# capnproto/capnproto-rust

Measured on AMD Instinct MI355X. Metric: GiB/s packed encode+decode, device-resident segments; % HBM roofline, higher is better.
Workload: dtype u8; 1 GPU; config2: 1048576 segments x 1024 B per GPU, ~30 % zero words, pack+unpack round trip; segments_per_gpu=1048576, unpacked_bytes_per_gpu=1073741824, global_unpacked_bytes=1073741824, parallelism=shard1

## Files before the change

capnproto-rust_amd/csrc/capi.hip:

```cpp
#ifndef CAPNP_STATE_ALLOC
#define CAPNP_STATE_ALLOC 1
#endif
#include <hip/hip_runtime.h>

#include <stdint.h>
#include <stdio.h>
#include <string.h>

#include <algorithm>
#include <chrono>
#include <string>
#include <cmath>
#include <mutex>
#include <vector>

#include "../../include/capnp_packed.h"
#include "../../include/capnp_packed_bench.h"
#include "common.h"
#include "frame.h"

extern "C" hipError_t capnp_launch_pack(const uint64_t*, const uint64_t*, uint64_t, uint32_t,
                                        uint8_t*, uint64_t, uint64_t*, uint64_t*, uint32_t*,
                                        hipStream_t);
extern "C" hipError_t capnp_launch_pack_gap(const uint64_t*, const uint64_t*, uint64_t, uint32_t,
                                            uint8_t*, uint64_t, uint64_t*, uint64_t*,
                                            const uint32_t*, hipStream_t);
extern "C" uint32_t capnp_pack_tile_words(void);
extern "C" hipError_t capnp_launch_msg_gap(const uint64_t*, const uint64_t*, uint64_t, uint64_t,
                                           uint32_t*, uint32_t*, hipStream_t);
extern "C" hipError_t capnp_launch_msg_tables(const uint64_t*, const uint64_t*, uint64_t,
                                              const uint64_t*, uint8_t*, uint64_t, uint64_t*,
                                              hipStream_t);
extern "C" hipError_t capnp_msg_scan_bytes(uint64_t, size_t*);
extern "C" hipError_t capnp_launch_msg_prepare(const uint64_t*, const uint64_t*, const uint64_t*,
                                               uint64_t, uint64_t*, uint64_t*, uint64_t*,
                                               uint64_t*, void*, size_t, uint64_t*, uint64_t*,
                                               hipStream_t);
extern "C" hipError_t capnp_launch_msg_offsets(const uint64_t*, const uint64_t*, uint64_t,
                                               uint64_t*, hipStream_t);
extern "C" hipError_t capnp_launch_msg_frame(const uint8_t*, const uint64_t*, uint64_t, int,
                                             uint64_t, int, uint64_t*, uint64_t*, int32_t*,
                                             uint64_t*, void*, size_t, uint64_t*, uint64_t*,
                                             hipStream_t);
extern "C" hipError_t capnp_launch_msg_segs(const uint8_t*, const uint64_t*, uint64_t, int,
                                            uint64_t, int, const int32_t*, const uint64_t*,
                                            const uint64_t*, const uint64_t*, uint64_t*,
                                            uint64_t*, uint64_t*, hipStream_t);
extern "C" hipError_t capnp_launch_msg_status(uint64_t, const int32_t*, const uint64_t*,
                                              const int32_t*, const uint64_t*, int32_t*,
                                              uint64_t*, hipStream_t);
extern "C" hipError_t capnp_launch_flat_frame(const uint8_t*, const uint64_t*, uint64_t, int,
                                              uint64_t, int, uint64_t*, int32_t*, uint64_t*,
                                              uint64_t*, void*, size_t, uint64_t*, hipStream_t);
extern "C" hipError_t capnp_launch_flat_segs(const uint8_t*, const uint64_t*, uint64_t, int,
                                             uint64_t, int, const int32_t*, const uint64_t*,
                                             uint32_t*, hipStream_t);
extern "C" size_t capnp_pack_state_bytes(uint64_t, uint32_t);
extern "C" hipError_t capnp_launch_unpack(const uint8_t*, const uint64_t*, uint64_t, uint32_t,
                                          uint64_t*, const uint64_t*, int32_t*, uint64_t*,
                                          const uint32_t*, hipStream_t);
extern "C" hipError_t capnp_launch_gen(uint64_t*, const uint64_t*, uint64_t, uint64_t,
                                       const uint8_t*, uint32_t, uint32_t, hipStream_t);
extern "C" uint64_t capnp_carsales_plan(const uint32_t*, uint64_t, uint64_t, uint32_t*, uint64_t*,
                                        uint64_t);
extern "C" hipError_t capnp_launch_gen_carsales(uint64_t*, uint64_t, const uint32_t*,
                                                const uint64_t*, uint64_t, hipStream_t);
extern "C" size_t capnp_resync_ws_bytes(uint64_t n, uint64_t total_bytes);
extern "C" size_t capnp_msg_chain_ws_bytes(uint64_t words_cap);
extern "C" hipError_t capnp_resync_read_stream(const uint8_t*, uint64_t, uint64_t, uint64_t*,
                                               uint64_t*, uint64_t, uint64_t*, uint64_t*,
                                               uint64_t*, int*, void*, size_t, hipStream_t,
                                               uint64_t*);
extern "C" hipError_t capnp_launch_msg_meta(const uint64_t*, const uint64_t*, uint64_t, uint64_t,
                                            int, uint64_t*, uint64_t*, uint64_t*, hipStream_t);
extern "C" hipError_t capnp_launch_msg_seglist(const uint64_t*, const uint64_t*, uint64_t,
                                               const uint64_t*, uint64_t*, hipStream_t);
// ... 27 lines not shown
                                          uint64_t total_bytes, uint64_t* d_out,
                                          const uint64_t* d_out_off, int32_t* d_status,
                                          uint64_t* d_consumed, void* d_ws, size_t ws_bytes,
                                          hipStream_t s, int* passes, int* serial,
                                          const int32_t** failed_flag);
extern "C" hipError_t capnp_launch_msg_read(const uint8_t*, uint64_t, uint32_t, uint32_t, uint64_t,
                                            uint32_t, uint64_t, uint64_t, FrameResult*, uint64_t*,
                                            uint64_t*, uint32_t*, uint32_t, hipStream_t);
extern "C" uint32_t capnp_msg_pack_words(void);
extern "C" hipError_t capnp_launch_msg_pack(const uint64_t*, const uint64_t*, uint32_t, uint32_t,
                                            uint8_t*, uint64_t, uint64_t*, uint32_t*, uint32_t,
                                            uint8_t*, hipStream_t);
extern "C" hipError_t capnp_launch_frame(const uint8_t*, uint64_t, uint32_t, uint32_t, uint64_t,
                                         uint32_t, uint64_t, uint64_t, FrameResult*, hipStream_t);
extern "C" hipError_t capnp_launch_msg_read_service(const uint64_t*, uint64_t*, uint32_t, uint64_t,
                                                    FrameResult*, uint32_t*, hipStream_t);
extern "C" hipError_t capnp_launch_msg_pack_service(const uint64_t*, uint64_t*, uint32_t, uint64_t,
                                                    uint32_t*, hipStream_t);

namespace {

constexpr uint32_t kDefaultTileChunks = 16;
constexpr uint32_t kMaxTileChunks = 64;

size_t round16(size_t x) { return (x + 15) & ~size_t(15); }

}

constexpr size_t kTablePrefixBytes = 4096;
#ifndef PARALLEL_BODY_WORDS
#define PARALLEL_BODY_WORDS 65536
#endif
constexpr uint64_t kParallelBodyWords = PARALLEL_BODY_WORDS;

struct CallSvc {
    hipStream_t s = nullptr;
    uint64_t* h = nullptr;
    uint64_t* d = nullptr;
    uint64_t* line = nullptr;
    const uint64_t* line_d = nullptr;
    bool line_dev = false;
    uint64_t args[kSvcArgs] = {};
    uint64_t bell = 0;
    uint32_t gen = 0;
    bool live = false;
    std::chrono::steady_clock::time_point last{};
};

struct capnp_ctx {
    int device = 0;
    hipStream_t stream = nullptr;
    uint8_t* d_state = nullptr;
    size_t state_cap = 0;
    uint8_t* d_stage = nullptr;
    size_t stage_cap = 0;
    uint8_t* d_body = nullptr;
    size_t body_cap = 0;
    FrameResult* d_frame = nullptr;
    FrameResult* h_frame = nullptr;
    hipStream_t sstream[3] = {nullptr, nullptr, nullptr};
    hipEvent_t ev_in[2] = {}, ev_comp[2] = {}, ev_off[2] = {}, ev_out[2] = {};
    uint8_t* d_slot[2] = {nullptr, nullptr};
    size_t slot_cap = 0;
    uint64_t* h_slot_off[2] = {nullptr, nullptr};
    size_t h_slot_off_cap = 0;
    uint8_t* d_msg = nullptr;
    size_t msg_cap = 0;
    uint8_t* d_resync = nullptr;
    size_t resync_cap = 0;
    uint8_t* d_wt = nullptr;
    size_t wt_cap = 0;
    uint8_t* d_pwt = nullptr;
    size_t pwt_cap = 0;
    uint8_t* d_stream_words = nullptr;
    size_t stream_words_cap = 0;
    int resync_passes = 0, resync_serial = 0;
    const int32_t* resync_failed = nullptr;
    hipStream_t resync_stream = nullptr;
    hipEvent_t ev_resync = nullptr;
    uint32_t* d_bad = nullptr;
    uint32_t* h_bad = nullptr;
    uint8_t* h_pin = nullptr;
    uint8_t* d_pin = nullptr;
    size_t pin_cap = 0;
    FrameResult* d_hframe = nullptr;
    uint8_t* d_req = nullptr;
    int req_ok = -1;
    uint32_t* h_flag = nullptr;
    uint32_t* d_flag = nullptr;
    uint32_t call_seq = 0;
    CallSvc svc[2];
    std::chrono::steady_clock::time_point percall_last{};
    bool percall_any = false;
    static constexpr int kUseSlots = 8;
    hipStream_t use_s[kUseSlots] = {};
    hipEvent_t use_ev[kUseSlots] = {};
    int use_next = 0;
    std::string err;
};

constexpr size_t kPinnedCall = size_t(4) << 20;
#ifndef WRITE_PIN_MAX
#define WRITE_PIN_MAX kPinnedCall
#endif
constexpr size_t kWritePinMax = WRITE_PIN_MAX;

// ... 27 lines not shown
}

#define HIP_TRY(expr)                                   \
    do {                                                \
        hipError_t e_ = (expr);                         \
        if (e_ != hipSuccess) return fail(ctx, e_, #expr); \
    } while (0)

hipStream_t pick(capnp_ctx*, void* s) { return (hipStream_t)s; }

void mark_use(capnp_ctx* ctx, hipStream_t s) {
    if (s == ctx->stream) return;
    hipStreamCaptureStatus cs = hipStreamCaptureStatusNone;
    if (hipStreamIsCapturing(s, &cs) != hipSuccess || cs != hipStreamCaptureStatusNone) return;
    int k = 0;
    while (k < capnp_ctx::kUseSlots && !(ctx->use_ev[k] && ctx->use_s[k] == s)) k++;
    if (k == capnp_ctx::kUseSlots) {
        k = ctx->use_next;
        ctx->use_next = (k + 1) % capnp_ctx::kUseSlots;
        if (ctx->use_ev[k]) {
            (void)hipEventSynchronize(ctx->use_ev[k]);
        } else if (hipEventCreateWithFlags(&ctx->use_ev[k], hipEventDisableTiming) != hipSuccess) {
            ctx->use_ev[k] = nullptr;
            (void)hipStreamSynchronize(s);
            return;
        }
    }
    ctx->use_s[k] = s;
    if (hipEventRecord(ctx->use_ev[k], s) != hipSuccess) (void)hipStreamSynchronize(s);
}

struct UseMark {
    capnp_ctx* ctx;
    hipStream_t s;
    ~UseMark() {
        if (ctx) mark_use(ctx, s);
    }
};

void svc_stop_all(capnp_ctx* ctx);

hipError_t wait_uses(capnp_ctx* ctx) {
    svc_stop_all(ctx);
    hipError_t e = hipSuccess, r;
    if (ctx->stream && (r = hipStreamSynchronize(ctx->stream)) != hipSuccess) e = r;
    for (int k = 0; k < capnp_ctx::kUseSlots; k++)
        if (ctx->use_ev[k] && ctx->use_s[k] && (r = hipEventSynchronize(ctx->use_ev[k])) != hipSuccess)
            e = r;
    for (int k = 0; k < 3; k++)
        if (ctx->sstream[k] && (r = hipStreamSynchronize(ctx->sstream[k])) != hipSuccess) e = r;
    return e;
}

capnp_status ensure_state(capnp_ctx* ctx, size_t bytes) {
    if (bytes <= ctx->state_cap) return CAPNP_OK;
    HIP_TRY(hipSetDevice(ctx->device));
    if (ctx->d_state) {
        HIP_TRY(wait_uses(ctx));
        HIP_TRY(hipFree(ctx->d_state));
        ctx->d_state = nullptr;
        ctx->state_cap = 0;
    }
    size_t cap = std::max<size_t>(bytes, 1 << 16);
#if CAPNP_STATE_ALLOC == 1
    HIP_TRY(hipExtMallocWithFlags(reinterpret_cast<void**>(&ctx->d_state), cap,
                                  hipDeviceMallocUncached));
#elif CAPNP_STATE_ALLOC == 2
    HIP_TRY(hipExtMallocWithFlags(reinterpret_cast<void**>(&ctx->d_state), cap,
                                  hipDeviceMallocFinegrained));
#else
    HIP_TRY(hipMalloc(&ctx->d_state, cap));
#endif
    ctx->state_cap = cap;
    return CAPNP_OK;
}

capnp_status settle_resync(capnp_ctx* ctx) {
    if (!ctx->resync_failed) return CAPNP_OK;
    int32_t f = 0;
    HIP_TRY(hipStreamSynchronize(ctx->resync_stream));
    HIP_TRY(hipMemcpy(&f, ctx->resync_failed, 4, hipMemcpyDeviceToHost));
    if (f) ctx->resync_serial = 3;
    ctx->resync_failed = nullptr;
    return CAPNP_OK;
}

capnp_status ensure_buf(capnp_ctx* ctx, uint8_t** buf, size_t* cap_io, size_t bytes) {
    if (buf == &ctx->d_resync) {
        const capnp_status st = settle_resync(ctx);
        if (st != CAPNP_OK) return st;
    }
    if (bytes <= *cap_io) return CAPNP_OK;
    HIP_TRY(hipSetDevice(ctx->device));
    if (*buf) {
        HIP_TRY(wait_uses(ctx));
        HIP_TRY(hipFree(*buf));
        *buf = nullptr;
        *cap_io = 0;
    }
    size_t cap = std::max<size_t>(round16(bytes) + 64, 1 << 20);
    HIP_TRY(hipMalloc(buf, cap));
    *cap_io = cap;
    return CAPNP_OK;
}

capnp_status ensure_stage(capnp_ctx* ctx, size_t bytes) {
    return ensure_buf(ctx, &ctx->d_stage, &ctx->stage_cap, bytes);
}

capnp_status ensure_pin(capnp_ctx* ctx, size_t bytes) {
    if (bytes <= ctx->pin_cap) return CAPNP_OK;
    HIP_TRY(hipSetDevice(ctx->device));
    if (ctx->h_pin) {
        svc_stop_all(ctx);
        HIP_TRY(hipStreamSynchronize(ctx->stream));
        HIP_TRY(hipHostFree(ctx->h_pin));
        ctx->h_pin = nullptr;
        ctx->pin_cap = 0;
    }
    const size_t cap = std::max<size_t>(round16(bytes) + 64, 1 << 16);
    HIP_TRY(hipHostMalloc(&ctx->h_pin, cap, 0));
    ctx->pin_cap = cap;
    void* dp = nullptr;
    HIP_TRY(hipHostGetDevicePointer(&dp, ctx->h_pin, 0));
    ctx->d_pin = static_cast<uint8_t*>(dp);
    return CAPNP_OK;
// ... 235 lines not shown

size_t state_bytes_for(size_t nchunks, uint32_t tc) {
    return capnp_pack_state_bytes(nchunks, tc) + 16;
}

uint32_t tile_chunks_for(uint64_t total_words, size_t n) {
    if (n == 0) return kDefaultTileChunks;
    const double mean = (double)total_words / (double)n;
    const double steps = std::max(1.0, std::ceil(mean / 64.0));
    double t = (double)(capnp_pack_tile_words() / 64) / steps;
    uint32_t tc = (uint32_t)std::max(1.0, std::min(t, (double)kMaxTileChunks));
    return tc;
}

bool force_word_tiles() {
    static const bool v = [] {
        const char* e = getenv("CAPNP_WORD_TILES");
        return e && e[0] == '1';
    }();
    return v;
}

constexpr uint64_t kWordTileMean = 512;
constexpr uint64_t kLongUnitsMin = 256;
constexpr uint64_t kLongUnitWords = 2048;
constexpr uint64_t kBlockDecodeWords = 32768;

capnp_status pack_batch_dev(capnp_ctx* ctx, const uint64_t* d_words, const uint64_t* d_off,
                            size_t n, uint8_t* d_out, size_t cap, uint64_t* d_out_off,
                            uint32_t tc, hipStream_t s, uint32_t* d_sync = nullptr,
                            const uint64_t* host_wr = nullptr) {
    if (n > 0 && !d_off) return CAPNP_E_INVALID_ARGUMENT;
    if (!d_out_off) return CAPNP_E_INVALID_ARGUMENT;
    UseMark um{ctx, s};
    if (tc == 0 && n > 0) {
        uint64_t wr[2];
        if (host_wr) {
            wr[0] = host_wr[0];
            wr[1] = host_wr[1];
        } else {
            capnp_status vst = check_offsets(ctx, s, {{d_off, n, ~0ull}});
            if (vst != CAPNP_OK) return vst;
            wr[0] = checked_ends(ctx, 0)[0];
            wr[1] = checked_ends(ctx, 0)[1];
        }
        if (wr[1] < wr[0]) return CAPNP_E_INVALID_ARGUMENT;
        const uint64_t words = wr[1] - wr[0];
        if (words && (words / n >= kWordTileMean || force_word_tiles())) {
            const uint64_t ntiles = capnp_pack_wt_tiles(wr[0], wr[1]);
            capnp_status st = ensure_state(ctx, capnp_pack_state_bytes(ntiles, 1) + 16);
            if (st != CAPNP_OK) return st;
            st = ensure_buf(ctx, &ctx->d_pwt, &ctx->pwt_cap, capnp_pack_wt_ws_bytes(wr[0], wr[1]));
            if (st != CAPNP_OK) return st;
            HIP_TRY(capnp_launch_pack_wt(d_words, d_off, n, d_out, cap, d_out_off,
                                         reinterpret_cast<uint64_t*>(ctx->d_state), ctx->d_pwt,
                                         ctx->pwt_cap, d_sync, wr[0], wr[1], s));
            return CAPNP_OK;
        }
        tc = tile_chunks_for(words, n);
    }
    if (tc == 0) tc = kDefaultTileChunks;
    if (tc > kMaxTileChunks) return CAPNP_E_INVALID_ARGUMENT;
    const size_t sb = state_bytes_for(n, tc);
    capnp_status st = ensure_state(ctx, sb);
    if (st != CAPNP_OK) return st;
    HIP_TRY(capnp_launch_pack(d_words, d_off, n, tc, d_out, cap, d_out_off,
                              reinterpret_cast<uint64_t*>(ctx->d_state), d_sync, s));
    return CAPNP_OK;
}

capnp_status pack_host(capnp_ctx* ctx, const uint64_t* words, const uint64_t* off, size_t n,
                       uint8_t* out, size_t out_cap, uint64_t* out_off_host, uint64_t* total) {
    const uint64_t base = n ? off[0] : 0;
    const uint64_t nw = n ? off[n] - base : 0;
    std::vector<uint64_t> rel(n + 1);
    for (size_t i = 0; i <= n; i++) {
        rel[i] = n ? off[i] - base : 0;
        if (i && off[i] < off[i - 1]) return CAPNP_E_INVALID_ARGUMENT;
    }
    const uint64_t wr[2] = {0, nw};
    const size_t bound = capnp_packed_batch_bound_bytes(nw, n);
    const size_t o_words = 0;
    const size_t o_off = round16(nw * 8);
    const size_t o_oo = o_off + round16((n + 1) * 8);
    const size_t o_out = o_oo + round16((n + 1) * 8);
    capnp_status st = ensure_stage(ctx, o_out + bound + 16);
    if (st != CAPNP_OK) return st;
    uint8_t* d = ctx->d_stage;
    hipStream_t s = ctx->stream;
    const uint32_t tc = (n && nw / n >= kWordTileMean) ? 0u : tile_chunks_for(nw, n);
    if (o_out + bound <= kPinnedCall) {
        st = ensure_pin(ctx, o_out + bound + 16);
        if (st != CAPNP_OK) return st;
        uint8_t* h = ctx->h_pin;
        if (nw) memcpy(h + o_words, words + base, nw * 8);
        memcpy(h + o_off, rel.data(), (n + 1) * 8);
        HIP_TRY(hipMemcpyAsync(d, h, o_oo, hipMemcpyHostToDevice, s));
        st = pack_batch_dev(ctx, reinterpret_cast<uint64_t*>(d + o_words),
                            reinterpret_cast<uint64_t*>(d + o_off), n, d + o_out, bound,
                            reinterpret_cast<uint64_t*>(d + o_oo), tc, s, nullptr, wr);
        if (st != CAPNP_OK) return st;
        HIP_TRY(hipMemcpyAsync(h + o_oo, d + o_oo, o_out - o_oo + bound, hipMemcpyDeviceToHost, s));
        HIP_TRY(hipStreamSynchronize(s));
        const uint64_t* oo = reinterpret_cast<const uint64_t*>(h + o_oo);
        *total = oo[n];
        const size_t ncopy = std::min<uint64_t>(oo[n], out_cap);
        if (ncopy) memcpy(out, h + o_out, ncopy);
        if (out_off_host) memcpy(out_off_host, oo, (n + 1) * 8);
        return oo[n] > out_cap ? CAPNP_E_BUFFER_NOT_LARGE_ENOUGH : CAPNP_OK;
    }
    if (nw) HIP_TRY(hipMemcpyAsync(d + o_words, words + base, nw * 8, hipMemcpyHostToDevice, s));
    HIP_TRY(hipMemcpyAsync(d + o_off, rel.data(), (n + 1) * 8, hipMemcpyHostToDevice, s));
    st = pack_batch_dev(ctx, reinterpret_cast<uint64_t*>(d + o_words),
                        reinterpret_cast<uint64_t*>(d + o_off), n, d + o_out, bound,
                        reinterpret_cast<uint64_t*>(d + o_oo), tc, s, nullptr, wr);
    if (st != CAPNP_OK) return st;
    std::vector<uint64_t> oo(n + 1);
    HIP_TRY(hipMemcpyAsync(oo.data(), d + o_oo, (n + 1) * 8, hipMemcpyDeviceToHost, s));
    HIP_TRY(hipStreamSynchronize(s));
    *total = oo[n];
// ... 634 lines not shown
        HIP_TRY(hipEventRecord(ctx->ev_comp[k], s_comp));
        HIP_TRY(hipStreamWaitEvent(s_out, ctx->ev_comp[k], 0));
        if (wi)
            HIP_TRY(hipMemcpyAsync(words + w0, d + o_out, wi * 8, hipMemcpyDeviceToHost, s_out));
        HIP_TRY(hipMemcpyAsync(status + c0, d + o_st, ni * 4, hipMemcpyDeviceToHost, s_out));
        if (consumed)
            HIP_TRY(hipMemcpyAsync(consumed + c0, d + o_cs, ni * 8, hipMemcpyDeviceToHost,
                                   s_out));
        HIP_TRY(hipEventRecord(ctx->ev_out[k], s_out));
    }
    HIP_TRY(hipStreamSynchronize(s_out));
    return CAPNP_OK;
}

capnp_status capnp_gpu_write_messages(capnp_ctx* ctx, const uint64_t* d_words,
                                      const uint64_t* d_seg_word_off,
                                      const uint64_t* d_msg_seg_off, size_t nmsg,
                                      size_t total_segs, size_t total_words, uint8_t* d_out,
                                      size_t out_cap, uint64_t* d_msg_byte_off, void* stream) {
    if (!ctx || !d_msg_byte_off || (nmsg && (!d_seg_word_off || !d_msg_seg_off)))
        return CAPNP_E_INVALID_ARGUMENT;
    hipStream_t s = pick(ctx, stream);
    UseMark um{ctx, s};
    if (nmsg == 0) {
        HIP_TRY(hipMemsetAsync(d_msg_byte_off, 0, sizeof(uint64_t), s));
        return CAPNP_OK;
    }
    if (total_segs < nmsg || (total_words && !d_words)) return CAPNP_E_INVALID_ARGUMENT;
    {
        capnp_status vst = check_offsets(ctx, s,
                                         {{d_msg_seg_off, nmsg, (uint64_t)total_segs},
                                          {d_seg_word_off, total_segs, (uint64_t)total_words}});
        if (vst != CAPNP_OK) return vst;
    }
    {
        const size_t g_gap = 0;
        const size_t g_cboff = g_gap + round16(total_segs * 4);
        const size_t g_flag = g_cboff + round16((total_segs + 1) * 8);
        capnp_status st = ensure_buf(ctx, &ctx->d_msg, &ctx->msg_cap, g_flag + 64);
        if (st != CAPNP_OK) return st;
        uint8_t* d = ctx->d_msg;
        uint32_t* gap = reinterpret_cast<uint32_t*>(d + g_gap);
        uint64_t* cboff = reinterpret_cast<uint64_t*>(d + g_cboff);
        uint32_t* flag = reinterpret_cast<uint32_t*>(d + g_flag);
        HIP_TRY(capnp_launch_msg_gap(d_seg_word_off, d_msg_seg_off, nmsg, total_segs, gap, flag,
                                     s));
        uint32_t h_flag = 1;
        HIP_TRY(hipMemcpyAsync(&h_flag, flag, 4, hipMemcpyDeviceToHost, s));
        HIP_TRY(hipStreamSynchronize(s));
        if (h_flag == 0) {
            const uint32_t tc = tile_chunks_for(total_words, total_segs);
            st = ensure_state(ctx, state_bytes_for(total_segs, tc));
            if (st != CAPNP_OK) return st;
            HIP_TRY(capnp_launch_pack_gap(d_words, d_seg_word_off, total_segs, tc, d_out, out_cap,
                                          cboff, reinterpret_cast<uint64_t*>(ctx->d_state), gap,
                                          s));
            HIP_TRY(capnp_launch_msg_tables(d_seg_word_off, d_msg_seg_off, nmsg, cboff, d_out,
                                            out_cap, d_msg_byte_off, s));
            return CAPNP_OK;
        }
    }
    const size_t max_words = total_words + 2 * nmsg + total_segs / 2 + 1;
    const size_t max_chunks = 2 * nmsg + total_segs;
    size_t scan_bytes = 0;
    HIP_TRY(capnp_msg_scan_bytes(nmsg + 1, &scan_bytes));
    const size_t o_cw = 0;
    const size_t o_cc = o_cw + round16((nmsg + 1) * 8);
    const size_t o_wofs = o_cc + round16((nmsg + 1) * 8);
    const size_t o_cofs = o_wofs + round16((nmsg + 1) * 8);
    const size_t o_tmp = o_cofs + round16((nmsg + 1) * 8);
    const size_t o_coff = o_tmp + round16(scan_bytes + 16);
    const size_t o_cboff = o_coff + round16((max_chunks + 1) * 8);
    const size_t o_stage = o_cboff + round16((max_chunks + 1) * 8);
    capnp_status st = ensure_buf(ctx, &ctx->d_msg, &ctx->msg_cap, o_stage + max_words * 8 + 64);
    if (st != CAPNP_OK) return st;
    uint8_t* d = ctx->d_msg;
    auto U = [&](size_t o) { return reinterpret_cast<uint64_t*>(d + o); };
    HIP_TRY(capnp_launch_msg_prepare(d_words, d_seg_word_off, d_msg_seg_off, nmsg, U(o_cw),
                                     U(o_cc), U(o_wofs), U(o_cofs), d + o_tmp, scan_bytes,
                                     U(o_stage), U(o_coff), s));
    uint64_t tot[2] = {0, 0};
    HIP_TRY(hipMemcpyAsync(&tot[0], U(o_wofs) + nmsg, 8, hipMemcpyDeviceToHost, s));
    HIP_TRY(hipMemcpyAsync(&tot[1], U(o_cofs) + nmsg, 8, hipMemcpyDeviceToHost, s));
    HIP_TRY(hipStreamSynchronize(s));
    if (tot[0] > max_words || tot[1] > max_chunks) return CAPNP_E_INVALID_ARGUMENT;
    st = pack_batch_dev(ctx, U(o_stage), U(o_coff), tot[1], d_out, out_cap, U(o_cboff),
                        tile_chunks_for(tot[0], tot[1]), s);
    if (st != CAPNP_OK) return st;
    HIP_TRY(capnp_launch_msg_offsets(U(o_cofs), U(o_cboff), nmsg, d_msg_byte_off, s));
    return CAPNP_OK;
}

capnp_status capnp_gpu_read_messages(capnp_ctx* ctx, const uint8_t* d_packed,
                                     const uint64_t* d_msg_byte_off, size_t nmsg,
                                     const capnp_reader_options* opts, int try_mode,
                                     uint64_t* d_words, size_t words_cap,
                                     uint64_t* d_msg_word_off, uint64_t* d_seg_words,
                                     size_t segs_cap, uint64_t* d_msg_seg_off,
                                     int32_t* d_status, uint64_t* d_consumed, void* stream) {
    if (!ctx || !d_msg_word_off || !d_msg_seg_off ||
        (nmsg && (!d_msg_byte_off || !d_status)))
        return CAPNP_E_INVALID_ARGUMENT;
    hipStream_t s = pick(ctx, stream);
    UseMark um{ctx, s};
    if (nmsg == 0) {
        HIP_TRY(hipMemsetAsync(d_msg_word_off, 0, 8, s));
// ... 604 lines not shown
```

capnproto-rust_amd/csrc/pack.hip:

```cpp
#include "common.h"
#include <stdlib.h>
#include "../../include/capnp_packed.h"



#ifndef PACK_PROF
#define PACK_PROF 0
#endif
#if PACK_PROF
__device__ unsigned long long g_prof[8];
__device__ uint64_t* g_trace;
#define PROF_ADD(i, v) atomicAdd(&g_prof[i], (unsigned long long)(v))
#define TRACE(tile, k, v) do { if (g_trace) g_trace[(tile) * 8 + (k)] = (v); } while (0)
#define RT() __builtin_amdgcn_s_memrealtime()
#else
#define PROF_ADD(i, v) ((void)0)
#define TRACE(tile, k, v) ((void)0)
#define RT() 0ull
#endif

namespace {

constexpr int kWaves = 4;
constexpr int kThreads = kWaves * CAPNP_WAVE;
// ... 434 lines not shown
                b += 4;
                *reinterpret_cast<uint32_t*>(tab + b) = rel | (dd << 24);
            }
        }
    }
}

__device__ __forceinline__ void copy_out(const uint8_t* region, uint8_t* __restrict__ out,
                                         uint64_t D0, uint64_t len, uint64_t cap,
                                         uint32_t lane) {
    const uint64_t lo = D0;
    const uint64_t hi = (D0 + len < cap) ? D0 + len : cap;
    if (hi <= lo) return;
    const uint64_t a = (lo + 15) & ~15ull, b = hi & ~15ull;
    if (a > b) {
        if (lane < hi - lo) out[lo + lane] = region[lane];
        return;
    }
    if (lane < a - lo) out[lo + lane] = region[lane];
    const uint32_t m = (uint32_t)((a - D0) & 15);
    const uint32_t q = m >> 2, sb = m & 3;
    for (uint64_t blk = a + 16ull * lane; blk < b; blk += 16ull * CAPNP_WAVE) {
        const uint32_t s = (uint32_t)(blk - D0) & ~15u;
        const uint4 A = *reinterpret_cast<const uint4*>(region + s);
        const uint4 B = *reinterpret_cast<const uint4*>(region + s + 16);
        const uint32_t w[8] = {A.x, A.y, A.z, A.w, B.x, B.y, B.z, B.w};
        uint4 o;
        if (q == 0) {
            o = make_uint4(__builtin_amdgcn_alignbyte(w[1], w[0], sb),
                           __builtin_amdgcn_alignbyte(w[2], w[1], sb),
                           __builtin_amdgcn_alignbyte(w[3], w[2], sb),
                           __builtin_amdgcn_alignbyte(w[4], w[3], sb));
        } else if (q == 1) {
            o = make_uint4(__builtin_amdgcn_alignbyte(w[2], w[1], sb),
                           __builtin_amdgcn_alignbyte(w[3], w[2], sb),
                           __builtin_amdgcn_alignbyte(w[4], w[3], sb),
                           __builtin_amdgcn_alignbyte(w[5], w[4], sb));
        } else if (q == 2) {
            o = make_uint4(__builtin_amdgcn_alignbyte(w[3], w[2], sb),
                           __builtin_amdgcn_alignbyte(w[4], w[3], sb),
                           __builtin_amdgcn_alignbyte(w[5], w[4], sb),
                           __builtin_amdgcn_alignbyte(w[6], w[5], sb));
        } else {
            o = make_uint4(__builtin_amdgcn_alignbyte(w[4], w[3], sb),
                           __builtin_amdgcn_alignbyte(w[5], w[4], sb),
                           __builtin_amdgcn_alignbyte(w[6], w[5], sb),
                           __builtin_amdgcn_alignbyte(w[7], w[6], sb));
        }
        *reinterpret_cast<uint4*>(out + blk) = o;
    }
    if (lane < hi - b) out[b + lane] = region[(b - D0) + lane];
}

__device__ __forceinline__ void copy_out_tile(const uint8_t* region, uint8_t* __restrict__ out,
                                              uint64_t D0, uint64_t len, uint64_t cap,
                                              uint32_t lane, uint32_t wave) {
    const uint64_t lo = D0;
    const uint64_t hi = (D0 + len < cap) ? D0 + len : cap;
    if (hi <= lo) return;
    const uint64_t a = (lo + 15) & ~15ull, b = hi & ~15ull;
    if (a > b) {
        if (wave == 0 && lane < hi - lo) out[lo + lane] = region[lane];
        return;
    }
    if (wave == 0 && lane < a - lo) out[lo + lane] = region[lane];
    if (wave == kWaves - 1 && lane < hi - b) out[b + lane] = region[(b - D0) + lane];
    const uint32_t nb = (uint32_t)((b - a) >> 4);
    const uint32_t k0 = nb * wave / kWaves, k1 = nb * (wave + 1) / kWaves;
    const uint32_t m = (uint32_t)((a - D0) & 15);
    const uint32_t q = m >> 2, sb = m & 3;
    for (uint32_t k = k0 + lane; k < k1; k += CAPNP_WAVE) {
        const uint64_t blk = a + 16ull * k;
        const uint32_t s = (uint32_t)(blk - D0) & ~15u;
        const uint4 A = *reinterpret_cast<const uint4*>(region + s);
        const uint4 B = *reinterpret_cast<const uint4*>(region + s + 16);
        const uint32_t w[8] = {A.x, A.y, A.z, A.w, B.x, B.y, B.z, B.w};
        uint4 o;
        if (q == 0) {
            o = make_uint4(__builtin_amdgcn_alignbyte(w[1], w[0], sb),
                           __builtin_amdgcn_alignbyte(w[2], w[1], sb),
                           __builtin_amdgcn_alignbyte(w[3], w[2], sb),
                           __builtin_amdgcn_alignbyte(w[4], w[3], sb));
        } else if (q == 1) {
            o = make_uint4(__builtin_amdgcn_alignbyte(w[2], w[1], sb),
                           __builtin_amdgcn_alignbyte(w[3], w[2], sb),
                           __builtin_amdgcn_alignbyte(w[4], w[3], sb),
                           __builtin_amdgcn_alignbyte(w[5], w[4], sb));
        } else if (q == 2) {
            o = make_uint4(__builtin_amdgcn_alignbyte(w[3], w[2], sb),
                           __builtin_amdgcn_alignbyte(w[4], w[3], sb),
                           __builtin_amdgcn_alignbyte(w[5], w[4], sb),
                           __builtin_amdgcn_alignbyte(w[6], w[5], sb));
        } else {
            o = make_uint4(__builtin_amdgcn_alignbyte(w[4], w[3], sb),
                           __builtin_amdgcn_alignbyte(w[5], w[4], sb),
                           __builtin_amdgcn_alignbyte(w[6], w[5], sb),
                           __builtin_amdgcn_alignbyte(w[7], w[6], sb));
        }
        *reinterpret_cast<uint4*>(out + blk) = o;
    }
}

template <int MODE, uint32_t NWV = kWaves>
__device__ void run_streaming(const uint64_t* __restrict__ in, const uint64_t* off,
                              uint64_t* chunk_size, const uint64_t* chunk_pos, uint32_t nc,
                              uint32_t wave, uint32_t lane, uint8_t* ring, const Sel8* sel,
                              uint8_t* out, uint32_t mis, uint64_t out_cap,
                              const uint32_t* cgap, uint64_t* last_size = nullptr) {
    Packer pk;
    for (uint32_t ci = wave; ci < nc; ci += NWV) {
        const uint64_t woff = uniform64(off[ci]);
        const uint64_t len = uniform64(off[ci + 1]) - woff;
        const uint32_t g = cgap ? uniform(cgap[ci]) : 0u;
        if (len == 0) {
            if (MODE == MODE_SIZE && lane == 0) chunk_size[ci] = g;
            continue;
        }
        if (MODE == MODE_RING) {
            const uint64_t pos = lds_u64(&chunk_pos[ci]);
            if (pos + lds_u64(&chunk_size[ci]) > out_cap) continue;
            pk.begin(pos + g + mis);
        } else {
            pk.begin(0);
        }
        const uint64_t* src = in + woff;
        uint64_t wnext = lane < len ? src[lane] : 0;
        for (uint64_t base = 0;; base += 64) {
            const uint32_t nvalid = (uint32_t)((len - base) < 64 ? len - base : 64);
            const bool last = base + 64 >= len;
            const uint64_t w = wnext;
            if (!last) wnext = (base + 64 + lane < len) ? src[base + 64 + lane] : 0;
            pk.step<MODE>(w, nvalid, last, lane, ring, out, sel);
            if (last) break;
        }
        if (MODE == MODE_SIZE && lane == 0) chunk_size[ci] = pk.total + g;
        if (MODE == MODE_RING && last_size && ci + 1 == nc && lane == 0) *last_size = pk.total + g;
    }
}


constexpr uint32_t kWtRange = 64 * kStageSteps;
constexpr uint32_t kWtTile = kWaves * kWtRange;

struct LookbackArgs {
    uint64_t* ts;
    uint64_t* gs;
    uint64_t ntiles;
    const uint64_t* in;
    const uint64_t* chunk_off;
    uint64_t nchunks;
    uint32_t tc;
    const uint32_t* gap;
    uint32_t wt;
// ... 1287 lines not shown
        agg = scan_chunks32(sm, nc, lane);
        publish(LA, tile, agg, lane);
#if PACK_PROF == 3
        if (lane == 0) TRACE(tile, 2, RT());
#endif
    }
    const bool early_group = (tile % kGroup) == kGroup - 1;
    if (early_group && wave == kWaves - 1) {
        uint32_t a = 0;
#pragma unroll
        for (int w = 0; w < kWaves; w++) a += (uint32_t)lds_u64(&sm.wave_bytes[w]);
        publish_group_early(LA, tile, a, lane);
    }
    if (fits) {
        uint8_t* const region_m1 = (PACK_TILECOPY ? &sm.stage[0][0] + woff : region) - 1;
        const uint32_t t0 = (uint32_t)(k0 * kSyncWords - TW0);
        const __amdgpu_buffer_rsrc_t srs = __builtin_amdgcn_make_buffer_rsrc(
            SYNC ? sync + k0 : nullptr, 0, SYNC ? (int)((k1 - k0) * 4) : 0, 0x00020000);
#pragma unroll
        for (uint32_t s = 0; s < kCsSteps; s++) {
            const uint32_t oc = (uint32_t)__builtin_amdgcn_readlane((int)rec_oc, s);
            const uint32_t g = (uint32_t)__builtin_amdgcn_readlane((int)d_off, s);
            const uint32_t c = t0 - g;
            const uint32_t d = (c - lane) & (kSyncWords - 1);
            const uint32_t b = (lane + d - c) / (kSyncWords / 4u);
            cs_emit_word<SYNC>(clo[s], ilo[s], region_m1, sm.sel, srs, oc, d, b,
                               PACK_TILECOPY ? woff : 0u);
            cs_emit_word<SYNC>(chi[s], ihi[s], region_m1, sm.sel, srs, oc, d,
                               b + 64u / (kSyncWords / 4u), PACK_TILECOPY ? woff : 0u);
            __builtin_amdgcn_sched_barrier(0);
        }
    }
    if (wave == 0) {
#if PACK_PROF == 3
        wave_lds_sync();
        if (lane == 0) TRACE(tile, 3, RT());
#endif
#if PACK_ABL & 4
        const uint64_t excl = tile * 8800ull;
        (void)early_group;
#else
        const uint64_t excl = tile_offset(LA, tile, agg, lane, early_group);
#endif
#if PACK_PROF == 3
        if (lane == 0) TRACE(tile, 4, RT());
#endif
        if (lane < nc) sm.chunk_pos[lane] += excl;
        if (c1 == nchunks && lane == 0) out_off[nchunks] = excl + agg;
    }
    __syncthreads();
    for (uint32_t i = tid; i < nc; i += kThreads) out_off[c0 + i] = sm.chunk_pos[i];
    if (fits) {
        if (PACK_TILECOPY && !(PACK_ABL & 8)) {
            const uint32_t mis = (uint32_t)(reinterpret_cast<uintptr_t>(out) & 15u);
            const uint64_t D0 = lds_u64(&sm.chunk_pos[0]) + mis;
            copy_out_tile(&sm.stage[0][0], out - mis, D0, tbytes, out_cap + mis, lane, wave);
        } else if (nw && !(PACK_ABL & 8)) {
            const uint32_t mis = (uint32_t)(reinterpret_cast<uintptr_t>(out) & 15u);
            const uint64_t D0 = lds_u64(&sm.chunk_pos[wc0]) + mis;
            copy_out(region, out - mis, D0, lds_u64(&sm.wave_bytes[wave]), out_cap + mis, lane);
        }
#if PACK_PROF == 3
        __syncthreads();
        if (tid == 0) TRACE(tile, 5, RT());
#endif
    } else {
        if constexpr (SYNC)
            for (uint32_t i = tid; i < (uint32_t)(k1 - k0); i += kThreads) sync[k0 + i] = kSyncNone;
        if (tid == 0) ovf[tile] = 1;
    }
}

template <bool GAP>
__global__ void __launch_bounds__(kThreads)
pack_ovf_kernel(const uint64_t* __restrict__ in, const uint64_t* __restrict__ chunk_off,
                uint64_t nchunks, uint32_t tc, uint8_t* __restrict__ out, uint64_t out_cap,
                const uint64_t* __restrict__ out_off, const uint8_t* __restrict__ ovf,
                uint64_t ntiles, const uint32_t* __restrict__ gap) {
    __shared__ Smem<GAP> sm;
    __shared__ uint32_t lst[kThreads];
    __shared__ uint32_t nl;
    const uint32_t tid = threadIdx.x;
    const uint32_t lane = tid & 63u;
    const uint32_t wave = (uint32_t)__builtin_amdgcn_readfirstlane((int)(tid >> 6));
    for (uint32_t i = tid; i <= kSelCopy; i += kThreads) sm.sel[i] = kSel8Table.e[i];
    const uint32_t mis = (uint32_t)(reinterpret_cast<uintptr_t>(out) & 15u);
    uint8_t* const outa = out - mis;
    uint8_t* region = sm.stage[wave];
    for (uint64_t base = (uint64_t)blockIdx.x * kThreads; base < ntiles;
         base += (uint64_t)gridDim.x * kThreads) {
        if (tid == 0) nl = 0;
        __syncthreads();
        if (base + tid < ntiles && ovf[base + tid]) lst[atomicAdd(&nl, 1u)] = tid;
        __syncthreads();
        const uint32_t n = nl;
        for (uint32_t k = 0; k < n; k++) {
            const uint64_t c0 = (base + lst[k]) * tc;
            const uint64_t c1 = c0 + tc < nchunks ? c0 + tc : nchunks;
            const uint32_t nc = (uint32_t)(c1 - c0);
            __syncthreads();
            for (uint32_t j = tid; j < nc; j += kThreads) {
                sm.chunk_pos[j] = out_off[c0 + j];
                sm.chunk_size[j] = out_off[c0 + j + 1] - out_off[c0 + j];
                if constexpr (GAP) sm.chunk_gap[j] = gap[c0 + j];
            }
            __syncthreads();
            run_streaming<MODE_RING>(in, chunk_off + c0, sm.chunk_size, sm.chunk_pos, nc, wave,
                                     lane, region, sm.sel, outa, mis, out_cap,
                                     GAP ? sm.chunk_gap : nullptr);
        }
        __syncthreads();
    }
}


#ifndef PACK_WT_OCC
#define PACK_WT_OCC 8
#endif

struct WtSmem {
    Sel8 sel[kSelCopy + 1];
    uint64_t wave_bytes[kWaves];
    uint32_t lastcs[kWaves];
    uint64_t excl;
    uint32_t wcarry[kWaves];
    uint32_t wext[kWaves];
    alignas(16) uint32_t pad[4];
    alignas(16) uint8_t stage[kWaves][kRegion];
};

__device__ __forceinline__ void size_step_s(StageState& pk, uint64_t w, uint32_t nvalid,
                                            uint64_t Sm, uint32_t lane, StepInfo& si) {
    const uint32_t tag = word_tag_dot((uint32_t)w, (uint32_t)(w >> 32));
    const uint32_t pop = __builtin_popcount(tag);
    const bool isz = tag == 0, isf = tag == 0xFF;
    const uint64_t V = low_mask(nvalid);
    const uint64_t Zm = ballot64(isz) & V;
    const uint64_t Lm = ballot64(pop >= 7) & V;
    const uint64_t Fm = ballot64(isf) & V;
    const StepMasks sm = resolve_step_s(Zm, Lm, Fm, Sm, nvalid, pk.carry);
    const uint32_t hsize = 1u + pop + ((0x101u >> pop) & 1u);
    const uint32_t size = mask_sel(sm.H, hsize, isz ? 0u : 8u);
    const uint32_t incl = wave_incl_scan(size);
    si.H = sm.H;
    si.pos = pk.o_c + pk.total + incl - size;
    si.tag = tag;
    si.meta = nvalid | (sm.absorbed_carry << 16);
    pk.carry = sm.next;
    pk.total += (uint32_t)__builtin_amdgcn_readlane((int)incl, 63);
}

struct RangeExit {
    Carry c;
    uint32_t homog;
};
__device__ __forceinline__ RangeExit range_exit(const uint64_t (&w)[kStageSteps],
                                                uint32_t sbits, uint32_t nw, uint32_t lane) {
    uint32_t t[kStageSteps];
#pragma unroll
    for (uint32_t s = 0; s < kStageSteps; s++) t[s] = tag_of(w[s]);
    int ks = -1;
    uint32_t js = 0;
    bool allz = true, allf = true;
#pragma unroll
    for (int s = kStageSteps - 1; s >= 0; s--) {
// ... 626 lines not shown
    msg_pack_body(S, words, off, nchunks, nwords, out, out_cap, total, flag, seq, scratch);
}

__global__ void __launch_bounds__(kMsgThreads)
msg_pack_service(const uint64_t* line, uint64_t* mark, uint32_t gen, uint64_t idle_ticks,
                 uint32_t* flag) {
    __shared__ MsgPackSmem S;
    __shared__ SvcCmd cmd;
    const uint32_t tid = threadIdx.x;
    const uint32_t lane = tid & 63u;
    const uint32_t wave = (uint32_t)__builtin_amdgcn_readfirstlane((int)(tid >> 6));
    uint32_t last = 0;
    while (svc_next(line, cmd, gen, last, idle_ticks, wave, lane)) {
        const SvcPackReq& q = *reinterpret_cast<const SvcPackReq*>(cmd.a);
        const uint64_t nn = uniform64(q.counts);
        uint8_t* const out = reinterpret_cast<uint8_t*>(uniform64(q.out));
        msg_pack_body(S, reinterpret_cast<const uint64_t*>(uniform64(q.words)),
                      reinterpret_cast<const uint64_t*>(uniform64(q.off)), (uint32_t)nn,
                      (uint32_t)(nn >> 32), out, uniform64(q.out_cap),
                      reinterpret_cast<uint64_t*>(out - 16), flag, last,
                      reinterpret_cast<uint8_t*>(uniform64(q.scratch)));
        svc_prof_done(cmd, tid);
        __syncthreads();
    }
    svc_exit(mark, gen, tid);
}

}

extern "C" uint32_t capnp_pack_tile_words(void) { return kWaves * 64 * kStageSteps; }

static uint64_t level_record_count(uint64_t ntiles) {
    uint64_t total = 0;
    for (uint64_t n = ntiles; n > 1;) {
        n = (n + kGroup - 1) / kGroup;
        total += n;
    }
    return total ? total : 1;
}

extern "C" size_t capnp_pack_state_bytes(uint64_t nchunks, uint32_t tc) {
    const uint64_t ntiles = (nchunks + tc - 1) / tc;
    return ((ntiles + level_record_count(ntiles)) * 8 + ntiles + 15) & ~size_t(15);
}

static uint8_t* pack_ovf_flags(uint64_t* d_state, uint64_t ntiles) {
    return reinterpret_cast<uint8_t*>(d_state + ntiles + level_record_count(ntiles));
}
static dim3 pack_ovf_grid(uint64_t ntiles) {
    const uint64_t g = (ntiles + kThreads - 1) / kThreads;
    return dim3((uint32_t)(g < 1024 ? g : 1024));
}

extern "C" hipError_t capnp_launch_pack(const uint64_t* d_in, const uint64_t* d_chunk_off,
                                        uint64_t nchunks, uint32_t tc, uint8_t* d_out,
                                        uint64_t out_cap, uint64_t* d_out_off,
                                        uint64_t* d_state, uint32_t* d_sync,
                                        hipStream_t stream) {
    if (tc == 0 || tc > kMaxTileChunks) return hipErrorInvalidValue;
    const uint64_t ntiles = (nchunks + tc - 1) / tc;
    if (nchunks == 0) {
        return hipMemsetAsync(d_out_off, 0, sizeof(uint64_t), stream);
    }
    hipError_t e = hipMemsetAsync(d_state, 0, capnp_pack_state_bytes(nchunks, tc), stream);
    if (e != hipSuccess) return e;
    uint8_t* ovf = pack_ovf_flags(d_state, ntiles);
    if (tc == kWaves * kCsSteps) {
        if (d_sync)
            hipLaunchKernelGGL((pack_cs_kernel<true>), dim3((uint32_t)ntiles), dim3(kThreads), 0,
                               stream, d_in, d_chunk_off, nchunks, tc, d_out, out_cap, d_out_off,
                               d_state, d_state + ntiles, d_sync, ovf);
        else
            hipLaunchKernelGGL((pack_cs_kernel<false>), dim3((uint32_t)ntiles), dim3(kThreads),
                               0, stream, d_in, d_chunk_off, nchunks, tc, d_out, out_cap,
                               d_out_off, d_state, d_state + ntiles, d_sync, ovf);
    } else if (d_sync) {
        hipLaunchKernelGGL((pack_lean_kernel<true>), dim3((uint32_t)ntiles), dim3(kThreads), 0,
                           stream, d_in, d_chunk_off, nchunks, tc, d_out, out_cap, d_out_off,
                           d_state, d_state + ntiles, d_sync, ovf);
    } else {
        hipLaunchKernelGGL((pack_lean_kernel<false>), dim3((uint32_t)ntiles), dim3(kThreads), 0,
                           stream, d_in, d_chunk_off, nchunks, tc, d_out, out_cap, d_out_off,
                           d_state, d_state + ntiles, d_sync, ovf);
    }
    hipLaunchKernelGGL((pack_ovf_kernel<false>), pack_ovf_grid(ntiles), dim3(kThreads), 0, stream,
                       d_in, d_chunk_off, nchunks, tc, d_out, out_cap, d_out_off, ovf, ntiles,
                       nullptr);
    return hipGetLastError();
}

extern "C" hipError_t capnp_launch_pack_gap(const uint64_t* d_in, const uint64_t* d_chunk_off,
                                            uint64_t nchunks, uint32_t tc, uint8_t* d_out,
                                            uint64_t out_cap, uint64_t* d_out_off,
                                            uint64_t* d_state, const uint32_t* d_gap,
                                            hipStream_t stream) {
    if (tc == 0 || tc > kMaxTileChunks || !d_gap) return hipErrorInvalidValue;
    const uint64_t ntiles = (nchunks + tc - 1) / tc;
    if (nchunks == 0) return hipMemsetAsync(d_out_off, 0, sizeof(uint64_t), stream);
    hipError_t e = hipMemsetAsync(d_state, 0, capnp_pack_state_bytes(nchunks, tc), stream);
    if (e != hipSuccess) return e;
    uint8_t* ovf = pack_ovf_flags(d_state, ntiles);
    if (tc == kWaves * kCsSteps)
        hipLaunchKernelGGL((pack_cs_kernel<false, true>), dim3((uint32_t)ntiles), dim3(kThreads),
                           0, stream, d_in, d_chunk_off, nchunks, tc, d_out, out_cap, d_out_off,
                           d_state, d_state + ntiles, nullptr, ovf, d_gap);
    else
        hipLaunchKernelGGL((pack_kernel<false, true>), dim3((uint32_t)ntiles), dim3(kThreads), 0,
                           stream, d_in, d_chunk_off, nchunks, tc, d_out, out_cap, d_out_off,
                           d_state, d_state + ntiles, nullptr, d_gap, ovf);
    hipLaunchKernelGGL((pack_ovf_kernel<true>), pack_ovf_grid(ntiles), dim3(kThreads), 0, stream,
                       d_in, d_chunk_off, nchunks, tc, d_out, out_cap, d_out_off, ovf, ntiles,
                       d_gap);
    return hipGetLastError();
}

extern "C" uint64_t capnp_pack_wt_tiles(uint64_t wlo, uint64_t whi) {
    return whi > wlo ? (whi + kWtTile - 1) / kWtTile - wlo / kWtTile : 0;
}

static uint64_t wt_bits_words(uint64_t wlo, uint64_t whi) {
    return ((whi + 63) >> 6) - (wlo >> 6) + 16;
}

extern "C" size_t capnp_pack_wt_ws_bytes(uint64_t wlo, uint64_t whi) {
    const uint64_t nt = capnp_pack_wt_tiles(wlo, whi);
    return (nt * (kWaves + 1) + wt_bits_words(wlo, whi)) * 8 + (nt * kWaves + 1) * 4 + 64;
}

extern "C" uint32_t capnp_pack_wt_words(void) { return kWtTile; }

extern "C" int capnp_pack_wt_dbg(uint32_t* out) {
    (void)out;
    return -1;
}

extern "C" hipError_t capnp_launch_pack_wt(const uint64_t* d_in, const uint64_t* d_chunk_off,
                                           uint64_t nchunks, uint8_t* d_out, uint64_t out_cap,
                                           uint64_t* d_out_off, uint64_t* d_state, void* d_ws,
                                           size_t ws_bytes, uint32_t* d_sync, uint64_t wlo,
                                           uint64_t whi, hipStream_t stream) {
    const uint64_t ntiles = capnp_pack_wt_tiles(wlo, whi);
// ... 80 lines not shown
```

Before: 1333 GiB/s.

## Self-clean pack state in overflow kernel to skip per-call memset; simplify tile copy

The pack overflow kernel now zeroes the tile state records and overflow flags it consumed. The host tracks whether the state buffer is known clean and skips the per-launch hipMemsetAsync when it is. The tile copy-out loses the byte-realignment path with alignbyte and uses plain unaligned 16-byte vector stores, since the stage buffer is aligned at the tile's start. This saves a memset launch and its traffic per call, at the cost of extra clean-tracking state that could go stale across streams or graph capture, and of possibly slower unaligned global stores.

```diff
diff --git a/capnproto-rust_amd/csrc/capi.hip b/capnproto-rust_amd/csrc/capi.hip
--- a/capnproto-rust_amd/csrc/capi.hip
+++ b/capnproto-rust_amd/csrc/capi.hip
@@ -22,6 +22,10 @@
 extern "C" hipError_t capnp_launch_pack(const uint64_t*, const uint64_t*, uint64_t, uint32_t,
                                         uint8_t*, uint64_t, uint64_t*, uint64_t*, uint32_t*,
                                         hipStream_t);
+extern "C" hipError_t capnp_launch_pack_ex(const uint64_t*, const uint64_t*, uint64_t, uint32_t,
+                                           uint8_t*, uint64_t, uint64_t*, uint64_t*, uint32_t*,
+                                           int, hipStream_t);
+extern "C" int capnp_pack_leaves_state_clean(void);
 extern "C" hipError_t capnp_launch_pack_gap(const uint64_t*, const uint64_t*, uint64_t, uint32_t,
                                             uint8_t*, uint64_t, uint64_t*, uint64_t*,
                                             const uint32_t*, hipStream_t);
@@ -155,6 +159,10 @@
     hipStream_t stream = nullptr;
     uint8_t* d_state = nullptr;
     size_t state_cap = 0;
+    size_t state_clean = 0;
+    bool state_any = false;
+    bool state_untracked = false;
+    hipStream_t state_stream = nullptr;
     uint8_t* d_stage = nullptr;
     size_t stage_cap = 0;
     uint8_t* d_body = nullptr;
@@ -288,6 +296,15 @@
     return e;
 }
 
+void note_state_use(capnp_ctx* ctx, hipStream_t s) {
+    if (ctx->state_untracked) return;
+    hipStreamCaptureStatus cs = hipStreamCaptureStatusNone;
+    if (hipStreamIsCapturing(s, &cs) != hipSuccess || cs != hipStreamCaptureStatusNone) {
+        ctx->state_untracked = true;
+        ctx->state_clean = 0;
+    }
+}
+
 capnp_status ensure_state(capnp_ctx* ctx, size_t bytes) {
     if (bytes <= ctx->state_cap) return CAPNP_OK;
     HIP_TRY(hipSetDevice(ctx->device));
@@ -308,6 +325,11 @@
     HIP_TRY(hipMalloc(&ctx->d_state, cap));
 #endif
     ctx->state_cap = cap;
+    ctx->state_clean = 0;
+    HIP_TRY(hipMemset(ctx->d_state, 0, cap));
+    HIP_TRY(hipStreamSynchronize(nullptr));
+    ctx->state_clean = ctx->state_untracked ? 0 : cap;
+    ctx->state_any = true;
     return CAPNP_OK;
 }
 
@@ -649,6 +671,8 @@
             if (st != CAPNP_OK) return st;
             st = ensure_buf(ctx, &ctx->d_pwt, &ctx->pwt_cap, capnp_pack_wt_ws_bytes(wr[0], wr[1]));
             if (st != CAPNP_OK) return st;
+            note_state_use(ctx, s);
+            ctx->state_clean = 0;
             HIP_TRY(capnp_launch_pack_wt(d_words, d_off, n, d_out, cap, d_out_off,
                                          reinterpret_cast<uint64_t*>(ctx->d_state), ctx->d_pwt,
                                          ctx->pwt_cap, d_sync, wr[0], wr[1], s));
@@ -661,8 +685,23 @@
     const size_t sb = state_bytes_for(n, tc);
     capnp_status st = ensure_state(ctx, sb);
     if (st != CAPNP_OK) return st;
-    HIP_TRY(capnp_launch_pack(d_words, d_off, n, tc, d_out, cap, d_out_off,
-                              reinterpret_cast<uint64_t*>(ctx->d_state), d_sync, s));
+    note_state_use(ctx, s);
+    const size_t used = capnp_pack_state_bytes(n, tc);
+    const size_t was_clean = ctx->state_clean;
+    const bool clean = used <= was_clean && (ctx->state_any || ctx->state_stream == s);
+    ctx->state_clean = 0;
+    HIP_TRY(capnp_launch_pack_ex(d_words, d_off, n, tc, d_out, cap, d_out_off,
+                                 reinterpret_cast<uint64_t*>(ctx->d_state), d_sync, clean ? 1 : 0,
+                                 s));
+    if (n == 0) {
+        ctx->state_clean = was_clean;
+    } else {
+        ctx->state_clean = capnp_pack_leaves_state_clean() && !ctx->state_untracked
+                               ? (clean ? was_clean : used)
+                               : 0;
+        ctx->state_any = false;
+        ctx->state_stream = s;
+    }
     return CAPNP_OK;
 }
 
@@ -1403,6 +1442,8 @@
             const uint32_t tc = tile_chunks_for(total_words, total_segs);
             st = ensure_state(ctx, state_bytes_for(total_segs, tc));
             if (st != CAPNP_OK) return st;
+            note_state_use(ctx, s);
+            ctx->state_clean = 0;
             HIP_TRY(capnp_launch_pack_gap(d_words, d_seg_word_off, total_segs, tc, d_out, out_cap,
                                           cboff, reinterpret_cast<uint64_t*>(ctx->d_state), gap,
                                           s));
diff --git a/capnproto-rust_amd/csrc/pack.hip b/capnproto-rust_amd/csrc/pack.hip
--- a/capnproto-rust_amd/csrc/pack.hip
+++ b/capnproto-rust_amd/csrc/pack.hip
@@ -510,53 +510,24 @@
     if (lane < hi - b) out[b + lane] = region[(b - D0) + lane];
 }
 
+typedef uint32_t u32x4 __attribute__((ext_vector_type(4)));
+typedef u32x4 __attribute__((aligned(1))) u32x4_unaligned;
+
 __device__ __forceinline__ void copy_out_tile(const uint8_t* region, uint8_t* __restrict__ out,
                                               uint64_t D0, uint64_t len, uint64_t cap,
                                               uint32_t lane, uint32_t wave) {
     const uint64_t lo = D0;
     const uint64_t hi = (D0 + len < cap) ? D0 + len : cap;
     if (hi <= lo) return;
-    const uint64_t a = (lo + 15) & ~15ull, b = hi & ~15ull;
-    if (a > b) {
-        if (wave == 0 && lane < hi - lo) out[lo + lane] = region[lane];
-        return;
-    }
-    if (wave == 0 && lane < a - lo) out[lo + lane] = region[lane];
-    if (wave == kWaves - 1 && lane < hi - b) out[b + lane] = region[(b - D0) + lane];
-    const uint32_t nb = (uint32_t)((b - a) >> 4);
+    const uint32_t L = (uint32_t)(hi - lo);
+    const uint32_t nb = L >> 4;
     const uint32_t k0 = nb * wave / kWaves, k1 = nb * (wave + 1) / kWaves;
-    const uint32_t m = (uint32_t)((a - D0) & 15);
-    const uint32_t q = m >> 2, sb = m & 3;
+    uint8_t* const dst = out + lo;
     for (uint32_t k = k0 + lane; k < k1; k += CAPNP_WAVE) {
-        const uint64_t blk = a + 16ull * k;
-        const uint32_t s = (uint32_t)(blk - D0) & ~15u;
-        const uint4 A = *reinterpret_cast<const uint4*>(region + s);
-        const uint4 B = *reinterpret_cast<const uint4*>(region + s + 16);
-        const uint32_t w[8] = {A.x, A.y, A.z, A.w, B.x, B.y, B.z, B.w};
-        uint4 o;
-        if (q == 0) {
-            o = make_uint4(__builtin_amdgcn_alignbyte(w[1], w[0], sb),
-                           __builtin_amdgcn_alignbyte(w[2], w[1], sb),
-                           __builtin_amdgcn_alignbyte(w[3], w[2], sb),
-                           __builtin_amdgcn_alignbyte(w[4], w[3], sb));
-        } else if (q == 1) {
-            o = make_uint4(__builtin_amdgcn_alignbyte(w[2], w[1], sb),
-                           __builtin_amdgcn_alignbyte(w[3], w[2], sb),
-                           __builtin_amdgcn_alignbyte(w[4], w[3], sb),
-                           __builtin_amdgcn_alignbyte(w[5], w[4], sb));
-        } else if (q == 2) {
-            o = make_uint4(__builtin_amdgcn_alignbyte(w[3], w[2], sb),
-                           __builtin_amdgcn_alignbyte(w[4], w[3], sb),
-                           __builtin_amdgcn_alignbyte(w[5], w[4], sb),
-                           __builtin_amdgcn_alignbyte(w[6], w[5], sb));
-        } else {
-            o = make_uint4(__builtin_amdgcn_alignbyte(w[4], w[3], sb),
-                           __builtin_amdgcn_alignbyte(w[5], w[4], sb),
-                           __builtin_amdgcn_alignbyte(w[6], w[5], sb),
-                           __builtin_amdgcn_alignbyte(w[7], w[6], sb));
-        }
-        *reinterpret_cast<uint4*>(out + blk) = o;
-    }
+        const u32x4 v = *reinterpret_cast<const u32x4*>(region + 16u * k);
+        *reinterpret_cast<u32x4_unaligned*>(dst + 16u * k) = v;
+    }
+    if (wave == kWaves - 1 && lane < L - 16u * nb) dst[16u * nb + lane] = region[16u * nb + lane];
 }
 
 template <int MODE, uint32_t NWV = kWaves>
@@ -1950,9 +1921,8 @@
     for (uint32_t i = tid; i < nc; i += kThreads) out_off[c0 + i] = sm.chunk_pos[i];
     if (fits) {
         if (PACK_TILECOPY && !(PACK_ABL & 8)) {
-            const uint32_t mis = (uint32_t)(reinterpret_cast<uintptr_t>(out) & 15u);
-            const uint64_t D0 = lds_u64(&sm.chunk_pos[0]) + mis;
-            copy_out_tile(&sm.stage[0][0], out - mis, D0, tbytes, out_cap + mis, lane, wave);
+            copy_out_tile(&sm.stage[0][0], out, lds_u64(&sm.chunk_pos[0]), tbytes, out_cap, lane,
+                          wave);
         } else if (nw && !(PACK_ABL & 8)) {
             const uint32_t mis = (uint32_t)(reinterpret_cast<uintptr_t>(out) & 15u);
             const uint64_t D0 = lds_u64(&sm.chunk_pos[wc0]) + mis;
@@ -1969,12 +1939,16 @@
     }
 }
 
+#ifndef PACK_SELFCLEAN
+#define PACK_SELFCLEAN 1
+#endif
 template <bool GAP>
 __global__ void __launch_bounds__(kThreads)
 pack_ovf_kernel(const uint64_t* __restrict__ in, const uint64_t* __restrict__ chunk_off,
                 uint64_t nchunks, uint32_t tc, uint8_t* __restrict__ out, uint64_t out_cap,
-                const uint64_t* __restrict__ out_off, const uint8_t* __restrict__ ovf,
-                uint64_t ntiles, const uint32_t* __restrict__ gap) {
+                const uint64_t* __restrict__ out_off, uint8_t* __restrict__ ovf,
+                uint64_t ntiles, const uint32_t* __restrict__ gap,
+                uint64_t* __restrict__ rec = nullptr, uint64_t nrec = 0) {
     __shared__ Smem<GAP> sm;
     __shared__ uint32_t lst[kThreads];
     __shared__ uint32_t nl;
@@ -1989,7 +1963,10 @@
          base += (uint64_t)gridDim.x * kThreads) {
         if (tid == 0) nl = 0;
         __syncthreads();
-        if (base + tid < ntiles && ovf[base + tid]) lst[atomicAdd(&nl, 1u)] = tid;
+        if (base + tid < ntiles && ovf[base + tid]) {
+            lst[atomicAdd(&nl, 1u)] = tid;
+            if (nrec) ovf[base + tid] = 0;
+        }
         __syncthreads();
         const uint32_t n = nl;
         for (uint32_t k = 0; k < n; k++) {
@@ -2009,6 +1986,9 @@
         }
         __syncthreads();
     }
+    for (uint64_t i = (uint64_t)blockIdx.x * kThreads + tid; i < nrec;
+         i += (uint64_t)gridDim.x * kThreads)
+        rec[i] = 0;
 }
 
 
@@ -2741,19 +2721,24 @@
     return dim3((uint32_t)(g < 1024 ? g : 1024));
 }
 
-extern "C" hipError_t capnp_launch_pack(const uint64_t* d_in, const uint64_t* d_chunk_off,
-                                        uint64_t nchunks, uint32_t tc, uint8_t* d_out,
-                                        uint64_t out_cap, uint64_t* d_out_off,
-                                        uint64_t* d_state, uint32_t* d_sync,
-                                        hipStream_t stream) {
+extern "C" int capnp_pack_leaves_state_clean(void) { return PACK_SELFCLEAN ? 1 : 0; }
+
+extern "C" hipError_t capnp_launch_pack_ex(const uint64_t* d_in, const uint64_t* d_chunk_off,
+                                           uint64_t nchunks, uint32_t tc, uint8_t* d_out,
+                                           uint64_t out_cap, uint64_t* d_out_off,
+                                           uint64_t* d_state, uint32_t* d_sync,
+                                           int state_clean, hipStream_t stream) {
     if (tc == 0 || tc > kMaxTileChunks) return hipErrorInvalidValue;
     const uint64_t ntiles = (nchunks + tc - 1) / tc;
     if (nchunks == 0) {
         return hipMemsetAsync(d_out_off, 0, sizeof(uint64_t), stream);
     }
-    hipError_t e = hipMemsetAsync(d_state, 0, capnp_pack_state_bytes(nchunks, tc), stream);
-    if (e != hipSuccess) return e;
+    if (!state_clean) {
+        hipError_t e = hipMemsetAsync(d_state, 0, capnp_pack_state_bytes(nchunks, tc), stream);
+        if (e != hipSuccess) return e;
+    }
     uint8_t* ovf = pack_ovf_flags(d_state, ntiles);
+    const uint64_t nrec = PACK_SELFCLEAN ? ntiles + level_record_count(ntiles) : 0;
     if (tc == kWaves * kCsSteps) {
         if (d_sync)
             hipLaunchKernelGGL((pack_cs_kernel<true>), dim3((uint32_t)ntiles), dim3(kThreads), 0,
@@ -2774,8 +2759,17 @@
     }
     hipLaunchKernelGGL((pack_ovf_kernel<false>), pack_ovf_grid(ntiles), dim3(kThreads), 0, stream,
                        d_in, d_chunk_off, nchunks, tc, d_out, out_cap, d_out_off, ovf, ntiles,
-                       nullptr);
+                       nullptr, d_state, nrec);
     return hipGetLastError();
+}
+
+extern "C" hipError_t capnp_launch_pack(const uint64_t* d_in, const uint64_t* d_chunk_off,
+                                        uint64_t nchunks, uint32_t tc, uint8_t* d_out,
+                                        uint64_t out_cap, uint64_t* d_out_off,
+                                        uint64_t* d_state, uint32_t* d_sync,
+                                        hipStream_t stream) {
+    return capnp_launch_pack_ex(d_in, d_chunk_off, nchunks, tc, d_out, out_cap, d_out_off,
+                                d_state, d_sync, 0, stream);
 }
 
 extern "C" hipError_t capnp_launch_pack_gap(const uint64_t* d_in, const uint64_t* d_chunk_off,
```

New measurement: 1349 GiB/s (median of 6 runs). 1.01x the previous value.
